# TIERS/multi-modal-loam

Hardware: AMD Instinct MI355X
Metric: scans/s (feature-extract+kNN+10 GN iters) on 16-ring x1800 + Livox 24k fused cloud (higher is better)
Workload: dtype f32/f64; 1 GPU; BASELINE configs[1]: fused VLP-16 16x1800 + Livox Horizon 24000 scan (52800 pts), local map 200000 pts, 1 association pass (thres_dist 25), 10 GN iterations, W=1; resident_slots=8192, stream_lanes=2, distinct_scans=64, map_tiles_touched=43, map_tiles_complete=43, parallelism=scan-sharded x1, device=AMD Radeon Graphics, cus=256

## Files before the change

### multi-modal-loam_amd/csrc/capi.hip

```cpp
#include <math.h>
#include <stdarg.h>
#include <stdio.h>
#include <stdlib.h>
#include <string.h>

#include <algorithm>

#include "mml_internal.h"

int mml_launch_detect_line(mml_ctx* ctx, int n, uint16_t* d_final);

namespace {

constexpr int kPackMaxSlots = 16;
constexpr size_t kStageDoubles = 1u << 22;

double* stage_alloc(mml_ctx* ctx, size_t doubles) {
    if (ctx->stage_cursor + doubles > ctx->h_stage_doubles) {
        mml_sync_all(ctx);
        ctx->stage_cursor = 0;
    }
    double* p = ctx->h_stage + ctx->stage_cursor;
    ctx->stage_cursor += (doubles + 7) & ~size_t(7);
    return p;
// ... 5 lines not shown
    if (e != hipSuccess) return e;
    ctx->cus = prop.multiProcessorCount;
    ctx->n_lanes = 2;
    if (const char* v = getenv("MML_LANES")) {
        const int n = atoi(v);
        if (n >= 1 && n <= mml_ctx::MAX_LANES) ctx->n_lanes = n;
    }
    const auto off = [](const char* name) {
        const char* v = getenv(name);
        return v && atoi(v) == 0;
    };
    ctx->onepass_wanted = !off("MML_ASSIGN_ONEPASS");
    ctx->solve_wide = !off("MML_SOLVE_WIDE");
    ctx->use_graph = getenv("MML_NO_GRAPH") == nullptr;
    ctx->lazy_undistort = !off("MML_LAZY_UNDISTORT");
    return hipSuccess;
}

}

double* mml_stage_alloc(mml_ctx* ctx, size_t doubles) { return stage_alloc(ctx, doubles); }

int mml_refuse(mml_ctx* ctx, int code, const char* fmt, ...) {
    if (ctx) {
        char m[192];
        va_list ap;
        va_start(ap, fmt);
        vsnprintf(m, sizeof(m), fmt, ap);
        va_end(ap);
        ctx->err = m;
// ... 79 lines not shown
    if (ctx->cfg.cell_surf <= 0) ctx->cfg.cell_surf = 5.0f * ctx->cfg.leaf_surf;
    if (ctx->cfg.max_features <= 0) ctx->cfg.max_features = 8192;
    if (ctx->cfg.max_map_points <= 0) ctx->cfg.max_map_points = 1 << 21;
    ctx->B = cfg->max_scans;
    ctx->NV = (cfg->max_velo_points + 63) & ~63;
    ctx->NL = (cfg->max_livox_points + 63) & ~63;
    ctx->NT = ctx->NV + ctx->NL;
    ctx->L = cfg->n_rings + cfg->n_livox_lines;
    ctx->MF = ctx->cfg.max_features;
    ctx->MM = ctx->cfg.max_map_points;
    ctx->VX_CAP = (int)ctx->NT;
    ctx->h_n_in.assign((size_t)ctx->B * 2, 0);
    ctx->raw_extracted.assign((size_t)ctx->B, 0);
    ctx->stats_stale.assign((size_t)ctx->B, 1);
    ctx->und_pending.assign((size_t)ctx->B, 0);
    auto fail = [&](hipError_t e, const char* what) {
        ctx->err = std::string(what) + ": " + hipGetErrorString(e);
        mml_destroy(ctx);
        return MML_ERR_HIP;
    };
    hipError_t e;
    if ((e = hipSetDevice(device)) != hipSuccess) return fail(e, "hipSetDevice");
    if ((e = read_settings(ctx)) != hipSuccess) return fail(e, "hipGetDeviceProperties");
    for (int l = 0; l < mml_ctx::MAX_LANES; ++l) {
        if ((e = hipStreamCreateWithFlags(&ctx->streams[l], hipStreamNonBlocking)) != hipSuccess)
            return fail(e, "hipStreamCreate");
        if ((e = hipEventCreateWithFlags(&ctx->lane_mark[l], hipEventDisableTiming)) != hipSuccess)
            return fail(e, "hipEventCreate");
    }
    if ((e = hipStreamCreateWithFlags(&ctx->copy_stream, hipStreamNonBlocking)) != hipSuccess) return fail(e, "hipStreamCreate");
// ... 650 lines not shown
int mml_cloud_download_registered(mml_ctx* ctx, int slot, const double* T_wl, uint8_t* out, int capacity_points, int* n_points) {
    return mml_cloud_download_registered_batch(ctx, slot, 1, T_wl, out, capacity_points, n_points);
}

int mml_cloud_upload(mml_ctx* ctx, int slot, const uint8_t* pointxyzinormal, int n_points, int n_velo) {
    CHECK_SLOTS(slot, 1);
    MML_REQUIRE(n_points >= 0 && n_velo >= 0 && n_velo <= n_points, MML_ERR_INVALID, "bad point counts");
    MML_REQUIRE(n_points == 0 || pointxyzinormal, MML_ERR_INVALID, "null point buffer");
    MML_REQUIRE(n_velo <= ctx->NV && n_points - n_velo <= ctx->NL, MML_ERR_CAPACITY,
                "cloud exceeds max_velo_points / max_livox_points (the Velodyne and Livox parts have their own regions)");
    const size_t bytes = (size_t)n_points * 48;
    int rc = ensure_wire_stage(ctx, bytes ? bytes : 48);
    if (rc != MML_OK) return rc;
    if (bytes) MML_HIP(hipMemcpyAsync(ctx->wire_stage.d, pointxyzinormal, bytes, hipMemcpyHostToDevice, MML_STREAM(ctx)));
    ctx->und_pending[slot] = 0;
    rc = mml_launch_cloud_decode(ctx, slot, reinterpret_cast<const float*>(ctx->wire_stage.d), n_points, n_velo);
    if (rc != MML_OK) return rc;
    MML_HIP(hipStreamSynchronize(MML_STREAM(ctx)));
    return MML_OK;
}

int mml_extract(mml_ctx* ctx, int first_slot, int count, const float* livox_extrinsic) {
    CHECK_SLOTS(first_slot, count);
    bool have = false;
    if (livox_extrinsic) {
        static const float I[16] = {1, 0, 0, 0, 0, 1, 0, 0, 0, 0, 1, 0, 0, 0, 0, 1};
        have = memcmp(I, livox_extrinsic, sizeof(I)) != 0;
        if (have) {
            double* st = stage_alloc(ctx, 8);
            memcpy(st, livox_extrinsic, sizeof(float) * 16);
// ... 1177 lines not shown
```

### multi-modal-loam_amd/csrc/feature.hip

```cpp
#include <math.h>

#include <algorithm>
#include <stdlib.h>

#include "libm_f32.h"
#include "mml_internal.h"

namespace {

enum : unsigned {
    A_W2 = 1u << 0,
    A_ANGLE = 1u << 1,
    A_CAND3 = 1u << 2,
    A_FAR = 1u << 3,
    A_REFL = 1u << 4,
    A_A3_SHIFT = 5,
    A_B3_SHIFT = 7,
    A_LFLAT = 1u << 9,
    A_RFLAT = 1u << 10,
    A_C150 = 1u << 11,
    A_F5_SHIFT = 12,
    A_NEAR = 1u << 14,
    A_VIS = 1u << 15
};
// ... 131 lines not shown
    }
    return ((unsigned long long)mhi << 32) | mlo;
}

typedef float v4f_nt __attribute__((ext_vector_type(4)));
__device__ __forceinline__ float4 nt_load4(const float4* p) {
    const v4f_nt v = __builtin_nontemporal_load(reinterpret_cast<const v4f_nt*>(p));
    return make_float4(v.x, v.y, v.z, v.w);
}

struct AssignAux {
    int first_finite, last_finite, trig, kept_velo;
    float startOri, endOri;
    int kept_livox, pad;
};
__device__ __forceinline__ void crop_test(const FeatParams& P, float x, float y, float z, bool& keep, bool& near_ok) {
    const float near2 = P.near_th * P.near_th, far2 = P.far_th * P.far_th;
    const float dis = x * x + y * y + z * z;
    keep = !(dis < near2 || dis > far2);
    near_ok = !(dis < near2);
}

__global__ void k_assign_init(FeatParams P, int count) {
    const int t = blockIdx.x * blockDim.x + threadIdx.x;
    if (t == 0) {
        P.sel_list_cnt[2 * P.first] = 0;
        P.sel_list_cnt[2 * P.first + 1] = 0;
    }
    if (t < count) {
        AssignAux* a = reinterpret_cast<AssignAux*>(P.assign_aux) + (P.first + t);
// ... 31 lines not shown
    const float guard = __builtin_fmaf(1.2e-4f, fabsf(inv_step), 2e-4f);
    const float rr = __builtin_fmaf(p.x, p.x, p.y * p.y);
    const float est = atan_est(p.z * __builtin_amdgcn_rsqf(rr)) * 57.29577951308232f;
    const float t = __builtin_fmaf(est - pitch0, inv_step, 0.5f);
    int scanID;
    if (fabsf(t - rintf(t)) > guard && fabsf(t) < 1e6f) {
        scanID = (int)t;
    } else {
        const float angle = (float)((double)(mml_libm::atanf_fd(p.z / sqrtf(p.x * p.x + p.y * p.y)) * 180.0f) / M_PI);
        const double v = (angle - pitch0) / pitch_step + 0.5;
        scanID = (v != v || v >= 2147483648.0 || v <= -2147483649.0) ? (-2147483647 - 1) : int(v);
    }
    return (scanID > (R - 1) || scanID < 0) ? 255 : scanID;
}

__device__ __forceinline__ float neg_atan2f(float y, float x) { return -mml_libm::atan2f_fd(y, x); }
__device__ __forceinline__ void sweep_azimuths(const float4 p0, const float4 p1, float& startOri, float& endOri) {
    startOri = neg_atan2f(p0.y, p0.x);
    endOri = (float)((double)neg_atan2f(p1.y, p1.x) + 2 * M_PI);
}

__global__ void k_libm_f32(const float* y, const float* x, long n, float* o2, float* o1) {
    const long i = (long)blockIdx.x * blockDim.x + threadIdx.x;
    if (i >= n) return;
    if (o2) o2[i] = mml_libm::atan2f_fd(y[i], x[i]);
    if (o1) o1[i] = mml_libm::atanf_fd(y[i]);
}

template <int PPT>
__global__ __launch_bounds__(AB_THREADS) void k_assign_a(FeatParams P) {
    __shared__ int s_bcnt[MAX_LINES];
// ... 285 lines not shown
    if (lane == 0) s_wvalid[wave] = __popcll(km);
    __syncthreads();
    if (!valid) return;
    const AssignAux* a = &aux;
    int pos = s_cnt[key] + __popcll(eq & lt);
    int fdst = (sensor == 0 ? 0 : a->kept_velo) + s_cnt[MAX_LINES + 1] + __popcll(km & lt);
    for (int w = 0; w < wave; ++w) {
        pos += s_wcnt[w][key];
        fdst += s_wvalid[w];
    }
    const int dst = s_ls[key] + pos;
    const size_t g = (size_t)b * P.NT + dst;
    P.ln_pts[g] = praw;
    float rel;
    if (sensor == 0) {
        const float startOri = a->startOri, endOri = a->endOri;
        float ori = P.raw_ori[(size_t)b * P.NV + i];
        if (i <= a->trig) {
            if (ori < startOri - M_PI / 2)
                ori += 2 * M_PI;
            else if (ori > startOri + M_PI * 3 / 2)
                ori -= 2 * M_PI;
        } else {
            ori += 2 * M_PI;
            if (ori < endOri - M_PI * 3 / 2)
                ori += 2 * M_PI;
            else if (ori > endOri + M_PI / 2)
                ori -= 2 * M_PI;
        }
        rel = (ori - startOri) / (endOri - startOri);
    } else {
        const mml_livox_point* in = P.livox_in + (size_t)b * P.NL;
        const double timeSpan = livox_to_sec(in[n - 1].offset_time);
        rel = livox_to_sec(off_time) / timeSpan;
    }
    P.ln_gidx[g] = keep ? fdst : ((sensor == 1 && near_ok) ? -2 : -1);
    P.ln_rel[g] = __float_as_int(rel);
}

#ifndef MML_CB_TP
#define MML_CB_TP 2
#endif
constexpr int CB_TP = MML_CB_TP;
constexpr int CB_THREADS = 1024;
constexpr int CB_TILE = CB_THREADS * CB_TP;
// ... 114 lines not shown
#pragma unroll
    for (int r = 0; r < CB_TP; ++r) {
        if (!valid[r]) continue;
        const int i = bx * CB_TILE + r * CB_THREADS + tid;
        const AssignAux* a = &aux;
        const int g = r * CB_WAVES + wave;
        const int sub = g / gpb;
        int pos = s_cnt[sub][key[r]] + rank[r];
        int fdst = (sensor == 0 ? 0 : a->kept_velo) + s_cnt[sub][MAX_LINES + 1] + krank[r];
        for (int w = sub * gpb; w < g; ++w) {
            pos += s_wcnt[w][key[r]];
            fdst += s_wvalid[w];
        }
        float rel;
        if (sensor == 0) {
            const float startOri = a->startOri, endOri = a->endOri;
            float o = ori[r];
            if (i <= a->trig) {
                if (o < startOri - M_PI / 2)
                    o += 2 * M_PI;
                else if (o > startOri + M_PI * 3 / 2)
                    o -= 2 * M_PI;
            } else {
                o += 2 * M_PI;
                if (o < endOri - M_PI * 3 / 2)
                    o += 2 * M_PI;
                else if (o > endOri + M_PI / 2)
                    o -= 2 * M_PI;
            }
            rel = (o - startOri) / (endOri - startOri);
        } else {
            rel = livox_to_sec(off_time[r]) / timeSpan;
        }
        const int e = s_kstart[key[r]] + (pos - s_cnt[0][key[r]]);
        s_pt[e] = praw[r];
        s_meta[e] = make_int2(keep[r] ? fdst : ((sensor == 1 && near_ok[r]) ? -2 : -1), __float_as_int(rel));
        s_dst[e] = s_ls[key[r]] + pos;
    }
    __syncthreads();
    const int nstaged = s_kstart[nkeys];
    for (int e = tid; e < nstaged; e += CB_THREADS) {
        const size_t g = (size_t)b * P.NT + s_dst[e];
        P.ln_pts[g] = s_pt[e];
        P.ln_gidx[g] = s_meta[e].x;
        P.ln_rel[g] = s_meta[e].y;
// ... 88 lines not shown
    return hipMemcpyFromSymbol(out, HIP_SYMBOL(g_op_dbg), sizeof(unsigned long long) * 16) == hipSuccess ? 0 : -1;
}
#else
#define OP_MARK(id)
#define OP_MARK0(id)
#endif
struct OnepassLds {
    int cnt[OP_GROUPS][OP_CSTRIDE];
    int gv[OP_GROUPS], gk[OP_GROUPS];
    int hist[OP_MAXKEYS + 2], koff[OP_MAXKEYS];
    int cond[OP_WAVES];
    int base[3];
    float ori[2];
    int out[2][MML_OP_BLK];
};
template <int SENSOR>
__device__ __forceinline__ void assign_onepass_body(const FeatParams& P, OnepassLds& S) {
    auto& s_cnt = S.cnt;
    auto& s_gv = S.gv;
    auto& s_gk = S.gk;
    auto& s_hist = S.hist;
    auto& s_koff = S.koff;
    auto& s_cond = S.cond;
    auto& s_base = S.base;
    auto& s_out = S.out;
    const int b = blockIdx.y + P.first, blk = blockIdx.x;
    const int tid = threadIdx.x, lane = tid & 63, wave = tid >> 6;
    const int i0 = blk * MML_OP_BLK;
#ifdef MML_OP_TIMING
    const bool op_dbg = SENSOR == 0 && tid == 64 && blk == MML_OP_TIMING && b == P.first + 517;
    const bool op_dbg0 = SENSOR == 0 && tid == 0 && blk == MML_OP_TIMING && b == P.first + 517;
    unsigned long long op_prev = clock64(), op_prev0 = op_prev;
// ... 10 lines not shown
        const mml_livox_point* in = P.livox_in + (size_t)b * P.NL;
#pragma unroll
        for (int r = 0; r < OP_PPT; ++r) {
            typedef unsigned lv_u4 __attribute__((ext_vector_type(4), aligned(4)));
            const unsigned* w = reinterpret_cast<const unsigned*>(in + min(i0 + r * OP_THREADS + tid, P.NL - 1));
            const lv_u4 head = *reinterpret_cast<const lv_u4*>(w);
            const unsigned tail = w[4];
            pt[r] = make_float4(__uint_as_float(head.y), __uint_as_float(head.z), __uint_as_float(head.w),
                                (float)(tail & 255u));
            xw[r] = head.x;
            info[r] = (tail >> 16) & 255u;
        }
    }
    const int n = P.n_in[2 * b + SENSOR];
    if (blk == 0 && tid == 0 && (SENSOR == 0 || P.n_in[2 * b] <= 0)) {
        P.slot_flags[2 * b] = 0;
        P.brk_cnt[b] = 0;
        P.redo_cnt[b] = 0;
    }
    if (i0 >= n) return;
    const int nkeys = SENSOR == 0 ? P.n_rings : P.n_lines;
    const int nbits = SENSOR == 0 ? P.ring_bits : P.line_bits;
    const int region = SENSOR == 0 ? 0 : P.NV;
    for (int k = tid; k < OP_GROUPS * OP_CSTRIDE; k += OP_THREADS) (&s_cnt[0][0])[k] = 0;
    if (SENSOR == 0 && wave == 0) {
        float so, eo;
        if (P.ends_inline) {
            sweep_ends(P, b, so, eo);
        } else {
            const AssignAux* a = reinterpret_cast<const AssignAux*>(P.assign_aux) + b;
            so = a->startOri;
            eo = a->endOri;
        }
        if (lane == 0) {
            S.ori[0] = so;
            S.ori[1] = eo;
        }
    }
    struct {
        float startOri, endOri;
    } aux;
    OP_MARK(0);
    __syncthreads();
    OP_MARK(1);
    aux.startOri = S.ori[0];
    aux.endOri = S.ori[1];
    const unsigned long long lt = (lane == 0) ? 0ull : (~0ull >> (64 - lane));
    int cond_min = 0x7fffffff;
#pragma unroll
    for (int r = 0; r < OP_PPT; ++r) {
        const int i = i0 + r * OP_THREADS + tid;
        bool valid = false, keep = false, near_ok = false, cond = false;
        int key = 0;
        if (i < n) {
            if constexpr (SENSOR == 0) {
                const float4 p = pt[r];
                float ori = 0.f;
                if (isfinite(p.x) && isfinite(p.y) && isfinite(p.z)) {
                    const int ring = velo_ring(p, P.pitch0, P.pitch_step, P.n_rings);
                    valid = ring != 255;
                    key = valid ? ring : 0;
                    ori = neg_atan2f(p.y, p.x);
                }
                xw[r] = __float_as_uint(ori);
                if (valid) {
                    float o = ori;
                    if (o < aux.startOri - M_PI / 2)
                        o += 2 * M_PI;
                    else if (o > aux.startOri + M_PI * 3 / 2)
                        o -= 2 * M_PI;
                    cond = o - aux.startOri > M_PI;
                }
            } else {
                const int line_num = (int)(info[r] & 255u);
                valid = !(line_num > nkeys - 1) && !(pt[r].x < 0.01);
                key = valid ? line_num : 0;
            }
            if (valid) crop_test(P, pt[r].x, pt[r].y, pt[r].z, keep, near_ok);
        }
        const unsigned long long eq = match_key(valid, key, nbits);
        const unsigned long long km = __ballot(keep), vm = __ballot(valid);
        const int g = r * OP_WAVES + wave;
        if (valid && (eq & lt) == 0) s_cnt[g][key] = __popcll(eq);
        if (lane == 0) {
            s_gv[g] = __popcll(vm);
            s_gk[g] = __popcll(km);
        }
// ... 104 lines not shown
    __syncthreads();
    OP_MARK(6);
    const int base_valid = region + s_base[0], base_keep = s_base[1], trig = s_base[2];
    double timeSpan = 1.0;
    if constexpr (SENSOR == 1) timeSpan = livox_to_sec(P.livox_in[(size_t)b * P.NL + n - 1].offset_time);
#pragma unroll
    for (int r = 0; r < OP_PPT; ++r) {
        const unsigned f = info[r];
        if (!(f & OPI_VALID)) continue;
        const int i = i0 + r * OP_THREADS + tid;
        const int key = (int)(f & 255u), g = r * OP_WAVES + wave;
        const int dst = base_valid + s_koff[key] + s_cnt[g][key] + (int)((f >> OPI_RANK_SHIFT) & 63u);
        const int fdst = base_keep + s_gk[g] + (int)((f >> OPI_KRANK_SHIFT) & 63u);
        float rel;
        if constexpr (SENSOR == 0) {
            const float startOri = aux.startOri, endOri = aux.endOri;
            float ori = __uint_as_float(xw[r]);
            if (i <= trig) {
                if (ori < startOri - M_PI / 2)
                    ori += 2 * M_PI;
                else if (ori > startOri + M_PI * 3 / 2)
                    ori -= 2 * M_PI;
            } else {
                ori += 2 * M_PI;
                if (ori < endOri - M_PI * 3 / 2)
                    ori += 2 * M_PI;
                else if (ori > endOri + M_PI / 2)
                    ori -= 2 * M_PI;
            }
            rel = (ori - startOri) / (endOri - startOri);
        } else {
            rel = livox_to_sec(xw[r]) / timeSpan;
        }
        const size_t gpos = (size_t)b * P.NT + dst;
        P.ln_pts[gpos] = pt[r];
        const bool keep = (f & OPI_KEEP) != 0;
        const int q = dst - base_valid;
        s_out[0][q] = keep ? fdst : ((SENSOR == 1 && (f & OPI_NEAR)) ? -2 : -1);
        s_out[1][q] = __float_as_int(rel);
        __builtin_amdgcn_sched_barrier(0);
    }
    OP_MARK(7);
    __syncthreads();
    OP_MARK(8);
    {
        const int tv = s_hist[nkeys];
        int* og = P.ln_gidx + (size_t)b * P.NT + base_valid;
        int* orl = P.ln_rel + (size_t)b * P.NT + base_valid;
        for (int k = tid; k < tv; k += OP_THREADS) {
            og[k] = s_out[0][k];
            orl[k] = s_out[1][k];
        }
    }
#ifdef MML_OP_TIMING
    asm volatile("s_waitcnt vmcnt(0)" ::: "memory");
    OP_MARK(9);
#endif
}

__global__ __launch_bounds__(OP_THREADS) void k_assign_onepass(FeatParams P) {
    __shared__ OnepassLds S;
    if (blockIdx.z == 0)
        assign_onepass_body<0>(P, S);
    else
        assign_onepass_body<1>(P, S);
}
template <int SENSOR>
__global__ __launch_bounds__(OP_THREADS) void k_assign_onepass_s(FeatParams P) {
    __shared__ OnepassLds S;
    assign_onepass_body<SENSOR>(P, S);
}

constexpr int TB_THREADS = 256;
__global__ __launch_bounds__(TB_THREADS) void k_assign_tables(FeatParams P, int count) {
    __shared__ int s_cum[64][MML_SEG_MAX + 1], s_pos[64][MML_SEG_MAX];
    __shared__ int s_nseg[64], s_len[64], s_rb[64];
    const int t = blockIdx.x;
    if (t >= count) return;
    const int b = P.first + t, tid = threadIdx.x;
    if (t == 0 && tid == 64) {
        P.sel_list_cnt[2 * P.first] = 0;
        P.sel_list_cnt[2 * P.first + 1] = 0;
    }
    if (tid < 64) {
        const int lane = tid;
// ... 2329 lines not shown
        return MML_ERR_HIP;
    float *dy = ty.d, *dx = tx.d, *d2 = t2.d, *d1 = t1.d;
    bool ok = hipMemcpy(dy, y, bytes, hipMemcpyHostToDevice) == hipSuccess && hipMemcpy(dx, x, bytes, hipMemcpyHostToDevice) == hipSuccess;
    if (ok) {
        hipLaunchKernelGGL(k_libm_f32, dim3((unsigned)((n + 255) / 256)), dim3(256), 0, MML_STREAM(ctx), dy, dx, n, d2, d1);
        ok = hipStreamSynchronize(MML_STREAM(ctx)) == hipSuccess;
    }
    if (ok && out_atan2) ok = hipMemcpy(out_atan2, d2, bytes, hipMemcpyDeviceToHost) == hipSuccess;
    if (ok && out_atan) ok = hipMemcpy(out_atan, d1, bytes, hipMemcpyDeviceToHost) == hipSuccess;
    return ok ? MML_OK : MML_ERR_HIP;
}

int mml_launch_extract(mml_ctx* ctx, int first, int count, bool have_extrinsic) {
    for (int i = 0; i < count; ++i) ctx->raw_extracted[first + i] = 1;
    for (int i = 0; i < count; ++i) ctx->und_pending[first + i] = 0;
    FeatParams P = make_params(ctx, first);
    P.extr = have_extrinsic ? ctx->d_extr : nullptr;
    hipStream_t s = MML_STREAM(ctx);
    if (ctx->onepass) {
        ctx->op_epoch = (ctx->op_epoch + 1) & 0x1ffffffu;
        if (ctx->op_epoch == 0) ctx->op_epoch = 1;
        P.op_epoch = ctx->op_epoch;
        const int nbv = (ctx->NV + MML_OP_BLK - 1) / MML_OP_BLK, nbl = (ctx->NL + MML_OP_BLK - 1) / MML_OP_BLK;
        P.ends_inline = count <= ST_SEGMENT_MAX_SLOTS ? 1 : 0;
        if (!P.ends_inline) {
            MmlStageScope t(ctx, "assign_ends");
            hipLaunchKernelGGL(k_assign_ends, dim3(count), dim3(64), 0, s, P, count);
        }
        {
            MmlStageScope t(ctx, "assign_onepass");
            const int nb = nbv > nbl ? nbv : nbl;
            if (P.ends_inline) {
                if (nb > 0) hipLaunchKernelGGL(k_assign_onepass, dim3(nb, count, nbl > 0 ? 2 : 1), dim3(OP_THREADS), 0, s, P);
            } else {
                if (nbv > 0) hipLaunchKernelGGL(k_assign_onepass_s<0>, dim3(nbv, count), dim3(OP_THREADS), 0, s, P);
                if (nbl > 0) hipLaunchKernelGGL(k_assign_onepass_s<1>, dim3(nbl, count), dim3(OP_THREADS), 0, s, P);
            }
        }
        {
            MmlStageScope t(ctx, "assign_tables");
            hipLaunchKernelGGL(k_assign_tables, dim3(count), dim3(TB_THREADS), 0, s, P, count);
        }
    } else {
    {
        MmlStageScope t(ctx, "assign_count");
        hipLaunchKernelGGL(k_assign_init, dim3((count + 255) / 256), dim3(256), 0, s, P, count);
        if (P.ab_ppt == 4)
            hipLaunchKernelGGL((k_assign_a<4>), dim3(P.nblk_max, count, 2), dim3(AB_THREADS), 0, s, P);
        else
            hipLaunchKernelGGL((k_assign_a<1>), dim3(P.nblk_max, count, 2), dim3(AB_THREADS), 0, s, P);
    }
    {
// ... 178 lines not shown
```

### multi-modal-loam_amd/csrc/mml_internal.h

```cpp
#ifndef MML_INTERNAL_H
#define MML_INTERNAL_H

#include <hip/hip_runtime.h>
#include <stdint.h>

#include <string>
#include <vector>

#include "mml_mem.h"
#include "mmloam_hip.h"

#define MML_WAVE 64

namespace mml_und {
__device__ __forceinline__ double sconst(double v) {
    asm("" : "+s"(v));
    return v;
}
}
#define MML_SEG_MAX 16
#define MML_OP_BLK 4096
#define MML_SEG_FLAT 512
#define MML_VOXEL_LDS_CAP 8192

// ... 57 lines not shown
    struct WinGraph {
        int first, count, W, max_iters, fixed;
        double huber, w_tan;
        hipStream_t stream;
        const double* Tbl;
        bool second;
        hipGraphExec_t exec;
    };
    std::vector<WinGraph> win_graphs;
    int device = 0;
    int cus = 0;
    bool onepass_wanted = true;
    bool solve_wide = true;
    bool use_graph = true;
    bool lazy_undistort = true;
    static constexpr int MAX_LANES = 8;
    hipStream_t streams[MAX_LANES] = {};
    hipStream_t copy_stream = nullptr;
    hipEvent_t lane_mark[MAX_LANES] = {};
    struct Upload {
        int first, count;
        hipEvent_t done;
    };
    std::vector<Upload> uploads;
    std::vector<hipEvent_t> upload_event_pool;
    int n_lanes = 1;
    int cur = 0;
    std::string err;
    MmlFixed fixed;

// ... 37 lines not shown
    unsigned* brk_queue = nullptr;
    int* brk_cnt = nullptr;
    int* queue_off = nullptr;
    unsigned* redo_queue = nullptr;
    uint8_t* sel_done = nullptr;
    int* sel_list = nullptr;
    int* sel_list_cnt = nullptr;
    unsigned char* st_exit = nullptr;
    int* vx_big = nullptr;

    int* cb_n = nullptr;

    uint8_t* ln_line = nullptr;
    int* slot_flags = nullptr;
    std::vector<char> und_pending;
    uint8_t* ln_label = nullptr;
    int* fu_info = nullptr;

    float4* ft_xyz[2] = {nullptr, nullptr};
    int* ft_n = nullptr;
    unsigned long long* vx_keys = nullptr;
    int* vx_gidx = nullptr;
    unsigned long long* seg_keys = nullptr;
    unsigned* seg_vals = nullptr;
    float4* seg_cat = nullptr;
    int* seg_flag = nullptr;
    int* seg_meta = nullptr;
    MmlGroup seg_scratch;
    MmlStaging<char, false> seg_tmp[8];
    int VX_CAP = 0;
// ... 116 lines not shown
int mml_stage_begin(mml_ctx* ctx, const char* name);
void mml_stage_end(mml_ctx* ctx, int token);
struct MmlStageScope {
    mml_ctx* c;
    int t;
    MmlStageScope(mml_ctx* ctx, const char* name) : c(ctx), t(mml_stage_begin(ctx, name)) {}
    ~MmlStageScope() { mml_stage_end(c, t); }
};

int mml_launch_extract(mml_ctx* ctx, int first, int count, bool have_extrinsic);
int mml_launch_cloud_decode(mml_ctx* ctx, int slot, const float* d_raw, int n, int n_velo);
int mml_launch_undistort(mml_ctx* ctx, int first, int count, const double* d_params);
int mml_launch_undistort_listed(mml_ctx* ctx, int first, int count, const double* d_params);
int mml_cloud_settle(mml_ctx* ctx, int first, int count);
#define MML_LABEL_SETTLED 0x40
int mml_launch_downsample(mml_ctx* ctx, int first, int count);
inline int mml_voxel_cap_corner(const mml_ctx* ctx) { return (ctx->NT > 65536 || MML_VOXEL_LDS_CAP < 2048) ? MML_VOXEL_LDS_CAP : 2048; }
int mml_build_grid(mml_ctx* ctx, int kind, const float* h_xyz, int m);
int mml_build_grid_device(mml_ctx* ctx, int kind, int m);
int mml_downsample_big(mml_ctx* ctx, int first, int count);
int mml_downsample_redo_overflow(mml_ctx* ctx, int first, int count, std::vector<int>* redone);
int mml_map_upkeep_increment(mml_ctx* ctx, int slot, const double* T_wl, int* n_out);
int mml_build_global_grid(mml_ctx* ctx, int kind, const float* h_xyz, const int* h_cube, int m, const int* cen);
int mml_build_global_grid_device(mml_ctx* ctx, int kind, const float4* d_pts, const uint16_t* d_tags, const int* d_cnt, int m,
                                 const int* cen);
int mml_cube_store_append(mml_ctx* ctx, int slot, const double* T_wl);
int mml_cube_store_increment(mml_ctx* ctx, const double* T_wl, int* n_out);
int mml_cube_store_download(mml_ctx* ctx, int kind, float* xyz, int* cube, int capacity, int* n, int* cen);
int mml_cube_store_reset(mml_ctx* ctx);
int mml_launch_knn5(mml_ctx* ctx, int kind, const float* d_q, int nq, float max_d2, int* d_idx, float* d_d2);
// ... 25 lines not shown
```

### multi-modal-loam_amd/csrc/undistort_dev.h

```cpp
#ifndef MML_UNDISTORT_DEV_H
#define MML_UNDISTORT_DEV_H
#include <hip/hip_runtime.h>
#include <math.h>

#include "mml_internal.h"

namespace mml_und {

struct Q4 {
    double x, y, z, w;
};
struct V3 {
    double x, y, z;
};
__device__ __forceinline__ V3 v3(double x, double y, double z) { return V3{x, y, z}; }
__device__ __forceinline__ V3 vcross(const V3& a, const V3& b) {
    return v3(a.y * b.z - a.z * b.y, a.z * b.x - a.x * b.z, a.x * b.y - a.y * b.x);
}
__device__ __forceinline__ double qdot(const Q4& a, const Q4& b) {
    return (a.x * b.x + a.z * b.z) + (a.y * b.y + a.w * b.w);
}
__device__ __forceinline__ Q4 qnormalized(const Q4& q) {
    double n = sqrt(qdot(q, q));
    return Q4{q.x / n, q.y / n, q.z / n, q.w / n};
// ... 149 lines not shown
```

### multi-modal-loam_amd/csrc/undistort_voxel.hip

```cpp
#include <math.h>

#include "mml_internal.h"
#include "undistort_dev.h"

namespace {
using namespace mml_und;

__global__ void k_undistort_prep(int count, const double* params, double* derived, double* par_keep, int* flags ) {
    const int s = blockIdx.x * blockDim.x + threadIdx.x;
    if (s >= count) return;
    for (int k = 0; k < 12; ++k) par_keep[12 * s + k] = params[12 * s + k];
    flags[2 * s + 1] = flags[2 * s];
    flags[2 * s] |= 2;
    const double* dR = params + 12 * s;
    const Q4 qlc = qnormalized(quat_from_matrix(dR));
    const double dd = (0.0 * qlc.x + 0.0 * qlc.z) + (0.0 * qlc.y + 1.0 * qlc.w);
    const double absD = fabs(dd);
    const double one = 1.0 - 2.220446049250313e-16;
    double theta = 0, sinTheta = 1;
    const bool linear = absD >= one;
    if (!linear) {
        theta = acos(absD);
        sinTheta = sin(theta);
    }
// ... 35 lines not shown
    __builtin_nontemporal_store(outv, pp);
}

constexpr int UND_LISTED_G = 8;
__device__ __forceinline__ int listed_position(const int* fu_info, const unsigned* lists, int list_stride, int NT, int b, int e) {
    const int nc = min(max(fu_info[8 * b + 6], 0), list_stride), ns = min(max(fu_info[8 * b + 7], 0), list_stride);
    if (e >= nc + ns) return -1;
    const int kind = e >= nc ? 1 : 0;
    const unsigned pos = lists[((size_t)b * 2 + kind) * list_stride + (e - (kind ? nc : 0))];
    return pos < (unsigned)NT ? (int)pos : -1;
}
__device__ __forceinline__ int listed_total(const int* fu_info, int list_stride, int b) {
    return min(max(fu_info[8 * b + 6], 0), list_stride) + min(max(fu_info[8 * b + 7], 0), list_stride);
}

__global__ __launch_bounds__(256) void k_undistort_listed(int first, int NT, int list_stride, const int* fu_info, const unsigned* lists,
                                                         float4* ln_pts, const int* ln_rel, const int* slot_flags, const double* params,
                                                         const double* derived) {
    const int b = blockIdx.y + first;
    const int n = listed_total(fu_info, list_stride, b);
    const bool time_is_one = (slot_flags[2 * b + 1] & 2) != 0;
    const double* dR = params + 12 * blockIdx.y;
    for (int e = blockIdx.x * 256 + threadIdx.x; e < n; e += UND_LISTED_G * 256) {
        const int pos = listed_position(fu_info, lists, list_stride, NT, b, e);
        if (pos < 0) continue;
        float4 p = ln_pts[(size_t)b * NT + pos];
        const float s = time_is_one ? 1.0f : __int_as_float(ln_rel[(size_t)b * NT + pos]);
        mml_und::undistort_point(dR, dR + 9, derived + 8 * blockIdx.y, s, p);
        ln_pts[(size_t)b * NT + pos] = p;
    }
}

__global__ __launch_bounds__(256) void k_settle_mark(int first, int NT, int list_stride, const int* fu_info, const unsigned* lists,
                                                    uint8_t* ln_label) {
    const int b = blockIdx.y + first;
    const int n = listed_total(fu_info, list_stride, b);
    for (int e = blockIdx.x * 256 + threadIdx.x; e < n; e += UND_LISTED_G * 256) {
        const int pos = listed_position(fu_info, lists, list_stride, NT, b, e);
        if (pos < 0) continue;
        uint8_t* lab = ln_label + (size_t)b * NT + pos;
        *lab = (uint8_t)(*lab | MML_LABEL_SETTLED);
    }
}

#ifdef MML_VX_TIMING
__device__ unsigned long long g_vx_dbg[16];
#define VX_MARK(id)                                    \
    do {                                               \
        if (vx_dbg) {                                  \
            const unsigned long long now_ = clock64(); \
            g_vx_dbg[id] += now_ - vx_prev;            \
            vx_prev = now_;                            \
        }                                              \
    } while (0)
extern "C" int mml_debug_vx_timing(unsigned long long* out, int reset) {
    if (reset) {
        unsigned long long z[16] = {};
// ... 370 lines not shown
    const int cap = blockIdx.y == 0 ? A.cap_y0 : A.cap_y1;
    if constexpr (LIST) {
        const int nbig = A.big[A.first];
        for (int e = blockIdx.x; e < nbig; e += gridDim.x) {
            voxel_slot<VX_THREADS>(A, S, keys, __builtin_amdgcn_readfirstlane(A.big[A.B + A.first + e]), kind, cap);
            __syncthreads();
        }
    } else {
        if (A.zero_big && blockIdx.x == 0 && blockIdx.y == 0 && threadIdx.x == 0) A.big[A.first] = 0;
        voxel_slot<VX_THREADS>(A, S, keys, (int)blockIdx.x + A.first, kind, cap);
    }
}

}

int mml_launch_undistort(mml_ctx* ctx, int first, int count, const double* d_params) {
    MmlStageScope t(ctx, "undistort");
    dim3 grid((ctx->NT + 255) / 256, count);
    hipLaunchKernelGGL(k_undistort_prep, dim3((count + 63) / 64), dim3(64), 0, MML_STREAM(ctx), count, d_params, ctx->d_und + 8 * (size_t)first,
                       ctx->d_und_par + 12 * (size_t)first, ctx->slot_flags + 2 * (size_t)first);
    hipLaunchKernelGGL(k_undistort<false>, grid, dim3(256), 0, MML_STREAM(ctx), first, ctx->NT, ctx->NV, ctx->cb_n, ctx->ln_pts,
                       ctx->ln_rel, ctx->slot_flags, d_params, ctx->d_und + 8 * (size_t)first, (uint8_t*)nullptr);
    MML_HIP(hipGetLastError());
    return MML_OK;
}

int mml_launch_undistort_listed(mml_ctx* ctx, int first, int count, const double* d_params) {
    MmlStageScope t(ctx, "undistort");
    for (int i = 0; i < count; ++i) ctx->und_pending[first + i] = 1;
    hipLaunchKernelGGL(k_undistort_prep, dim3((count + 63) / 64), dim3(64), 0, MML_STREAM(ctx), count, d_params, ctx->d_und + 8 * (size_t)first,
                       ctx->d_und_par + 12 * (size_t)first, ctx->slot_flags + 2 * (size_t)first);
    hipLaunchKernelGGL(k_undistort_listed, dim3(UND_LISTED_G, count), dim3(256), 0, MML_STREAM(ctx), first, ctx->NT, ctx->VX_CAP, ctx->fu_info,
                       reinterpret_cast<const unsigned*>(ctx->vx_keys), ctx->ln_pts, ctx->ln_rel, ctx->slot_flags, d_params,
                       ctx->d_und + 8 * (size_t)first);
    MML_HIP(hipGetLastError());
    return MML_OK;
}

int mml_cloud_settle(mml_ctx* ctx, int first, int count) {
    for (int i = 0; i < count;) {
        if (!ctx->und_pending[first + i]) {
            ++i;
            continue;
        }
        int n = 1;
        while (i + n < count && ctx->und_pending[first + i + n] && n < 32768) ++n;
        const int f = first + i;
        MmlStageScope t(ctx, "undistort_settle");
        hipLaunchKernelGGL(k_settle_mark, dim3(UND_LISTED_G, n), dim3(256), 0, MML_STREAM(ctx), f, ctx->NT, ctx->VX_CAP, ctx->fu_info,
                           reinterpret_cast<const unsigned*>(ctx->vx_keys), ctx->ln_label);
        hipLaunchKernelGGL(k_undistort<true>, dim3((ctx->NT + 255) / 256, n), dim3(256), 0, MML_STREAM(ctx), f, ctx->NT, ctx->NV, ctx->cb_n,
                           ctx->ln_pts, ctx->ln_rel, ctx->slot_flags, ctx->d_und_par + 12 * (size_t)f, ctx->d_und + 8 * (size_t)f, ctx->ln_label);
        MML_HIP(hipGetLastError());
        for (int k = 0; k < n; ++k) ctx->und_pending[f + k] = 0;
        i += n;
    }
    return MML_OK;
}

int mml_launch_downsample(mml_ctx* ctx, int first, int count) {
    MmlStageScope t(ctx, "voxel_downsample");
    for (int i = 0; i < count; ++i) ctx->stats_stale[first + i] = 1;
    if (ctx->NT > (1 << 20)) return mml_downsample_big(ctx, first, count);
    const int cap_surf = MML_VOXEL_LDS_CAP, cap_corner = mml_voxel_cap_corner(ctx);
    auto lds = [](int cap) { return (size_t)cap * sizeof(unsigned long long); };
    VoxelArgs A;
    A.first = first;
    A.NT = ctx->NT;
    A.MF = ctx->MF;
    A.B = ctx->B;
    A.list_stride = ctx->VX_CAP;
    A.fu_info = ctx->fu_info;
// ... 39 lines not shown
```

Before: 437,900 scans/s.

## Defer exact Velodyne azimuth and relative-time computation to undistortion points

In the one-pass ring assignment, a cheap polynomial atan2 estimate with reciprocal approximation decides the half-sweep flag. The exact atan2 is computed only when the estimate is near a decision boundary. Per-point relative time is no longer computed there; only the half-turn bit is stored and the slot is flagged as pending. The exact time is then computed lazily, only for listed points during undistortion, or in a new materialise kernel before full or settle undistortion. This removes exact atan2 work for every raw point at the cost of extra state, a flag protocol, and an added kernel on the settle path.

Result: no change. 440,900 scans/s (median of 6 runs) (+0.7%).

```diff
diff --git a/multi-modal-loam_amd/csrc/azimuth_est.h b/multi-modal-loam_amd/csrc/azimuth_est.h
--- /dev/null
+++ b/multi-modal-loam_amd/csrc/azimuth_est.h
@@ -0,0 +1,46 @@
+#pragma once
+#if defined(__HIPCC__)
+#define MML_AZI_HD __host__ __device__ inline __attribute__((always_inline))
+#else
+#define MML_AZI_HD inline
+#endif
+
+namespace mml_azi {
+
+constexpr float AZI_EST_ERR = 7.2e-7f;
+constexpr float AZI_GUARD = 4e-6f;
+
+MML_AZI_HD bool azimuth_est_defined(float y, float x) {
+    const float m = __builtin_fmaxf(__builtin_fabsf(x), __builtin_fabsf(y));
+    return m > 1e-18f && m < 1e18f;
+}
+
+template <class RCP>
+MML_AZI_HD float atan2f_est(float y, float x, RCP rcp) {
+    const float ax = __builtin_fabsf(x), ay = __builtin_fabsf(y);
+    const bool swap = ay > ax;
+    const float t = (swap ? ax : ay) * rcp(swap ? ay : ax);
+    const float z = t * t;
+    float p = -0.004054564982652664f;
+    p = __builtin_fmaf(p, z, 0.021862952038645744f);
+    p = __builtin_fmaf(p, z, -0.0559123232960701f);
+    p = __builtin_fmaf(p, z, 0.0964219719171524f);
+    p = __builtin_fmaf(p, z, -0.1390862911939621f);
+    p = __builtin_fmaf(p, z, 0.19946566224098206f);
+    p = __builtin_fmaf(p, z, -0.33329859375953674f);
+    p = __builtin_fmaf(p, z, 0.9999993443489075f);
+    float r = p * t;
+    r = swap ? 1.57079637f - r : r;
+    r = x < 0.0f ? 3.14159274f - r : r;
+    return __builtin_copysignf(r, y);
+}
+
+MML_AZI_HD bool half_turn_from_estimate(float est, float startOri, float t1, float t2, bool& cond) {
+    const float d1 = est - t1, d2 = est - t2;
+    const float w = est + (d1 < 0.0f ? 6.28318548f : (d2 > 0.0f ? -6.28318548f : 0.0f));
+    const float d3 = (w - startOri) - 3.14159274f;
+    cond = d3 > 0.0f;
+    return __builtin_fabsf(d1) > AZI_GUARD && __builtin_fabsf(d2) > AZI_GUARD && __builtin_fabsf(d3) > AZI_GUARD;
+}
+
+}
diff --git a/multi-modal-loam_amd/csrc/capi.hip b/multi-modal-loam_amd/csrc/capi.hip
--- a/multi-modal-loam_amd/csrc/capi.hip
+++ b/multi-modal-loam_amd/csrc/capi.hip
@@ -43,6 +43,10 @@
     ctx->solve_wide = !off("MML_SOLVE_WIDE");
     ctx->use_graph = getenv("MML_NO_GRAPH") == nullptr;
     ctx->lazy_undistort = !off("MML_LAZY_UNDISTORT");
+    {
+        const char* v = getenv("MML_EXACT_AZIMUTH");
+        ctx->exact_azimuth = v && atoi(v) != 0;
+    }
     return hipSuccess;
 }
 
@@ -152,6 +156,7 @@
     ctx->raw_extracted.assign((size_t)ctx->B, 0);
     ctx->stats_stale.assign((size_t)ctx->B, 1);
     ctx->und_pending.assign((size_t)ctx->B, 0);
+    ctx->azi_pending.assign((size_t)ctx->B, 0);
     auto fail = [&](hipError_t e, const char* what) {
         ctx->err = std::string(what) + ": " + hipGetErrorString(e);
         mml_destroy(ctx);
@@ -832,6 +837,7 @@
     if (rc != MML_OK) return rc;
     if (bytes) MML_HIP(hipMemcpyAsync(ctx->wire_stage.d, pointxyzinormal, bytes, hipMemcpyHostToDevice, MML_STREAM(ctx)));
     ctx->und_pending[slot] = 0;
+    ctx->azi_pending[slot] = 0;
     rc = mml_launch_cloud_decode(ctx, slot, reinterpret_cast<const float*>(ctx->wire_stage.d), n_points, n_velo);
     if (rc != MML_OK) return rc;
     MML_HIP(hipStreamSynchronize(MML_STREAM(ctx)));
diff --git a/multi-modal-loam_amd/csrc/feature.hip b/multi-modal-loam_amd/csrc/feature.hip
--- a/multi-modal-loam_amd/csrc/feature.hip
+++ b/multi-modal-loam_amd/csrc/feature.hip
@@ -1,10 +1,13 @@
 #include <math.h>
+#include <stddef.h>
 
 #include <algorithm>
 #include <stdlib.h>
 
+#include "azimuth_est.h"
 #include "libm_f32.h"
 #include "mml_internal.h"
+#include "undistort_dev.h"
 
 namespace {
 
@@ -169,6 +172,9 @@
     float startOri, endOri;
     int kept_livox, pad;
 };
+static_assert(offsetof(AssignAux, startOri) == 4 * MML_AUX_START_ORI && offsetof(AssignAux, endOri) == 4 * (MML_AUX_START_ORI + 1) &&
+                  sizeof(AssignAux) == 4 * MML_AUX_INTS,
+              "undistort_voxel.hip reads the sweep's two azimuths from assign_aux by these offsets");
 __device__ __forceinline__ void crop_test(const FeatParams& P, float x, float y, float z, bool& keep, bool& near_ok) {
     const float near2 = P.near_th * P.near_th, far2 = P.far_th * P.far_th;
     const float dis = x * x + y * y + z * z;
@@ -230,7 +236,8 @@
     return (scanID > (R - 1) || scanID < 0) ? 255 : scanID;
 }
 
-__device__ __forceinline__ float neg_atan2f(float y, float x) { return -mml_libm::atan2f_fd(y, x); }
+using mml_und::neg_atan2f;
+using mml_und::velo_rel_time;
 __device__ __forceinline__ void sweep_azimuths(const float4 p0, const float4 p1, float& startOri, float& endOri) {
     startOri = neg_atan2f(p0.y, p0.x);
     endOri = (float)((double)neg_atan2f(p1.y, p1.x) + 2 * M_PI);
@@ -546,21 +553,7 @@
     P.ln_pts[g] = praw;
     float rel;
     if (sensor == 0) {
-        const float startOri = a->startOri, endOri = a->endOri;
-        float ori = P.raw_ori[(size_t)b * P.NV + i];
-        if (i <= a->trig) {
-            if (ori < startOri - M_PI / 2)
-                ori += 2 * M_PI;
-            else if (ori > startOri + M_PI * 3 / 2)
-                ori -= 2 * M_PI;
-        } else {
-            ori += 2 * M_PI;
-            if (ori < endOri - M_PI * 3 / 2)
-                ori += 2 * M_PI;
-            else if (ori > endOri + M_PI / 2)
-                ori -= 2 * M_PI;
-        }
-        rel = (ori - startOri) / (endOri - startOri);
+        rel = velo_rel_time(P.raw_ori[(size_t)b * P.NV + i], i > a->trig, a->startOri, a->endOri);
     } else {
         const mml_livox_point* in = P.livox_in + (size_t)b * P.NL;
         const double timeSpan = livox_to_sec(in[n - 1].offset_time);
@@ -705,21 +698,7 @@
         }
         float rel;
         if (sensor == 0) {
-            const float startOri = a->startOri, endOri = a->endOri;
-            float o = ori[r];
-            if (i <= a->trig) {
-                if (o < startOri - M_PI / 2)
-                    o += 2 * M_PI;
-                else if (o > startOri + M_PI * 3 / 2)
-                    o -= 2 * M_PI;
-            } else {
-                o += 2 * M_PI;
-                if (o < endOri - M_PI * 3 / 2)
-                    o += 2 * M_PI;
-                else if (o > endOri + M_PI / 2)
-                    o -= 2 * M_PI;
-            }
-            rel = (o - startOri) / (endOri - startOri);
+            rel = velo_rel_time(ori[r], i > a->trig, a->startOri, a->endOri);
         } else {
             rel = livox_to_sec(off_time[r]) / timeSpan;
         }
@@ -838,8 +817,9 @@
     float ori[2];
     int out[2][MML_OP_BLK];
 };
-template <int SENSOR>
+template <int SENSOR, bool LAZY>
 __device__ __forceinline__ void assign_onepass_body(const FeatParams& P, OnepassLds& S) {
+    static_assert(SENSOR == 0 || !LAZY, "Livox records are not touched by the lazy azimuth");
     auto& s_cnt = S.cnt;
     auto& s_gv = S.gv;
     auto& s_gk = S.gk;
@@ -880,7 +860,7 @@
     }
     const int n = P.n_in[2 * b + SENSOR];
     if (blk == 0 && tid == 0 && (SENSOR == 0 || P.n_in[2 * b] <= 0)) {
-        P.slot_flags[2 * b] = 0;
+        P.slot_flags[2 * b] = LAZY ? MML_SLOT_AZI_PENDING : 0;
         P.brk_cnt[b] = 0;
         P.redo_cnt[b] = 0;
     }
@@ -901,6 +881,11 @@
         if (lane == 0) {
             S.ori[0] = so;
             S.ori[1] = eo;
+            if (LAZY && P.ends_inline && blk == 0) {
+                AssignAux* a = reinterpret_cast<AssignAux*>(P.assign_aux) + b;
+                a->startOri = so;
+                a->endOri = eo;
+            }
         }
     }
     struct {
@@ -911,6 +896,7 @@
     OP_MARK(1);
     aux.startOri = S.ori[0];
     aux.endOri = S.ori[1];
+    const float thr1 = (float)((double)aux.startOri - M_PI / 2), thr2 = (float)((double)aux.startOri + M_PI * 3 / 2);
     const unsigned long long lt = (lane == 0) ? 0ull : (~0ull >> (64 - lane));
     int cond_min = 0x7fffffff;
 #pragma unroll
@@ -926,17 +912,23 @@
                     const int ring = velo_ring(p, P.pitch0, P.pitch_step, P.n_rings);
                     valid = ring != 255;
                     key = valid ? ring : 0;
-                    ori = neg_atan2f(p.y, p.x);
+                    bool decided = false;
+                    if constexpr (LAZY) {
+                        const float est = -mml_azi::atan2f_est(p.y, p.x, [](float v) { return __builtin_amdgcn_rcpf(v); });
+                        decided = mml_azi::half_turn_from_estimate(est, aux.startOri, thr1, thr2, cond) && mml_azi::azimuth_est_defined(p.y, p.x);
+                    }
+                    if (!decided && (valid || !LAZY)) {
+                        ori = neg_atan2f(p.y, p.x);
+                        float o = ori;
+                        if (o < aux.startOri - M_PI / 2)
+                            o += 2 * M_PI;
+                        else if (o > aux.startOri + M_PI * 3 / 2)
+                            o -= 2 * M_PI;
+                        cond = o - aux.startOri > M_PI;
+                    }
+                    cond = cond && valid;
                 }
-                xw[r] = __float_as_uint(ori);
-                if (valid) {
-                    float o = ori;
-                    if (o < aux.startOri - M_PI / 2)
-                        o += 2 * M_PI;
-                    else if (o > aux.startOri + M_PI * 3 / 2)
-                        o -= 2 * M_PI;
-                    cond = o - aux.startOri > M_PI;
-                }
+                if constexpr (!LAZY) xw[r] = __float_as_uint(ori);
             } else {
                 const int line_num = (int)(info[r] & 255u);
                 valid = !(line_num > nkeys - 1) && !(pt[r].x < 0.01);
@@ -1071,21 +1063,10 @@
         const int fdst = base_keep + s_gk[g] + (int)((f >> OPI_KRANK_SHIFT) & 63u);
         float rel;
         if constexpr (SENSOR == 0) {
-            const float startOri = aux.startOri, endOri = aux.endOri;
-            float ori = __uint_as_float(xw[r]);
-            if (i <= trig) {
-                if (ori < startOri - M_PI / 2)
-                    ori += 2 * M_PI;
-                else if (ori > startOri + M_PI * 3 / 2)
-                    ori -= 2 * M_PI;
-            } else {
-                ori += 2 * M_PI;
-                if (ori < endOri - M_PI * 3 / 2)
-                    ori += 2 * M_PI;
-                else if (ori > endOri + M_PI / 2)
-                    ori -= 2 * M_PI;
-            }
-            rel = (ori - startOri) / (endOri - startOri);
+            if constexpr (LAZY)
+                rel = __int_as_float(i > trig ? 1 : 0);
+            else
+                rel = velo_rel_time(__uint_as_float(xw[r]), i > trig, aux.startOri, aux.endOri);
         } else {
             rel = livox_to_sec(xw[r]) / timeSpan;
         }
@@ -1115,17 +1096,18 @@
 #endif
 }
 
+template <bool LAZY>
 __global__ __launch_bounds__(OP_THREADS) void k_assign_onepass(FeatParams P) {
     __shared__ OnepassLds S;
     if (blockIdx.z == 0)
-        assign_onepass_body<0>(P, S);
+        assign_onepass_body<0, LAZY>(P, S);
     else
-        assign_onepass_body<1>(P, S);
-}
-template <int SENSOR>
+        assign_onepass_body<1, false>(P, S);
+}
+template <int SENSOR, bool LAZY = false>
 __global__ __launch_bounds__(OP_THREADS) void k_assign_onepass_s(FeatParams P) {
     __shared__ OnepassLds S;
-    assign_onepass_body<SENSOR>(P, S);
+    assign_onepass_body<SENSOR, LAZY>(P, S);
 }
 
 constexpr int TB_THREADS = 256;
@@ -3485,6 +3467,7 @@
 int mml_launch_extract(mml_ctx* ctx, int first, int count, bool have_extrinsic) {
     for (int i = 0; i < count; ++i) ctx->raw_extracted[first + i] = 1;
     for (int i = 0; i < count; ++i) ctx->und_pending[first + i] = 0;
+    for (int i = 0; i < count; ++i) ctx->azi_pending[first + i] = 0;
     FeatParams P = make_params(ctx, first);
     P.extr = have_extrinsic ? ctx->d_extr : nullptr;
     hipStream_t s = MML_STREAM(ctx);
@@ -3501,12 +3484,15 @@
         {
             MmlStageScope t(ctx, "assign_onepass");
             const int nb = nbv > nbl ? nbv : nbl;
+            const bool lazy = !ctx->exact_azimuth;
             if (P.ends_inline) {
-                if (nb > 0) hipLaunchKernelGGL(k_assign_onepass, dim3(nb, count, nbl > 0 ? 2 : 1), dim3(OP_THREADS), 0, s, P);
+                if (nb > 0) hipLaunchKernelGGL((lazy ? k_assign_onepass<true> : k_assign_onepass<false>), dim3(nb, count, nbl > 0 ? 2 : 1), dim3(OP_THREADS), 0, s, P);
             } else {
-                if (nbv > 0) hipLaunchKernelGGL(k_assign_onepass_s<0>, dim3(nbv, count), dim3(OP_THREADS), 0, s, P);
-                if (nbl > 0) hipLaunchKernelGGL(k_assign_onepass_s<1>, dim3(nbl, count), dim3(OP_THREADS), 0, s, P);
-            }
+                if (nbv > 0) hipLaunchKernelGGL((lazy ? k_assign_onepass_s<0, true> : k_assign_onepass_s<0, false>), dim3(nbv, count), dim3(OP_THREADS), 0, s, P);
+                if (nbl > 0) hipLaunchKernelGGL((k_assign_onepass_s<1, false>), dim3(nbl, count), dim3(OP_THREADS), 0, s, P);
+            }
+            if (lazy && nbv > 0)
+                for (int i = 0; i < count; ++i) ctx->azi_pending[first + i] = 1;
         }
         {
             MmlStageScope t(ctx, "assign_tables");
diff --git a/multi-modal-loam_amd/csrc/mml_internal.h b/multi-modal-loam_amd/csrc/mml_internal.h
--- a/multi-modal-loam_amd/csrc/mml_internal.h
+++ b/multi-modal-loam_amd/csrc/mml_internal.h
@@ -95,6 +95,7 @@
     bool solve_wide = true;
     bool use_graph = true;
     bool lazy_undistort = true;
+    bool exact_azimuth = false;
     static constexpr int MAX_LANES = 8;
     hipStream_t streams[MAX_LANES] = {};
     hipStream_t copy_stream = nullptr;
@@ -162,6 +163,7 @@
     uint8_t* ln_line = nullptr;
     int* slot_flags = nullptr;
     std::vector<char> und_pending;
+    std::vector<char> azi_pending;
     uint8_t* ln_label = nullptr;
     int* fu_info = nullptr;
 
@@ -308,6 +310,9 @@
 int mml_launch_undistort_listed(mml_ctx* ctx, int first, int count, const double* d_params);
 int mml_cloud_settle(mml_ctx* ctx, int first, int count);
 #define MML_LABEL_SETTLED 0x40
+#define MML_SLOT_AZI_PENDING 4
+#define MML_AUX_INTS 8
+#define MML_AUX_START_ORI 4
 int mml_launch_downsample(mml_ctx* ctx, int first, int count);
 inline int mml_voxel_cap_corner(const mml_ctx* ctx) { return (ctx->NT > 65536 || MML_VOXEL_LDS_CAP < 2048) ? MML_VOXEL_LDS_CAP : 2048; }
 int mml_build_grid(mml_ctx* ctx, int kind, const float* h_xyz, int m);
diff --git a/multi-modal-loam_amd/csrc/undistort_dev.h b/multi-modal-loam_amd/csrc/undistort_dev.h
--- a/multi-modal-loam_amd/csrc/undistort_dev.h
+++ b/multi-modal-loam_amd/csrc/undistort_dev.h
@@ -3,9 +3,30 @@
 #include <hip/hip_runtime.h>
 #include <math.h>
 
+#include "libm_f32.h"
 #include "mml_internal.h"
 
 namespace mml_und {
+
+__device__ __forceinline__ float velo_rel_time(float ori, bool half_passed, float startOri, float endOri) {
+    if (!half_passed) {
+        if (ori < startOri - M_PI / 2)
+            ori += 2 * M_PI;
+        else if (ori > startOri + M_PI * 3 / 2)
+            ori -= 2 * M_PI;
+    } else {
+        ori += 2 * M_PI;
+        if (ori < endOri - M_PI * 3 / 2)
+            ori += 2 * M_PI;
+        else if (ori > endOri + M_PI / 2)
+            ori -= 2 * M_PI;
+    }
+    return (ori - startOri) / (endOri - startOri);
+}
+__device__ __forceinline__ float neg_atan2f(float y, float x) { return -mml_libm::atan2f_fd(y, x); }
+__device__ __forceinline__ float velo_time_from_point(const float4& p, int half_bit, float startOri, float endOri) {
+    return velo_rel_time(neg_atan2f(p.y, p.x), half_bit != 0, startOri, endOri);
+}
 
 struct Q4 {
     double x, y, z, w;
diff --git a/multi-modal-loam_amd/csrc/undistort_voxel.hip b/multi-modal-loam_amd/csrc/undistort_voxel.hip
--- a/multi-modal-loam_amd/csrc/undistort_voxel.hip
+++ b/multi-modal-loam_amd/csrc/undistort_voxel.hip
@@ -73,18 +73,26 @@
     return min(max(fu_info[8 * b + 6], 0), list_stride) + min(max(fu_info[8 * b + 7], 0), list_stride);
 }
 
-__global__ __launch_bounds__(256) void k_undistort_listed(int first, int NT, int list_stride, const int* fu_info, const unsigned* lists,
-                                                         float4* ln_pts, const int* ln_rel, const int* slot_flags, const double* params,
-                                                         const double* derived) {
+__global__ __launch_bounds__(256) void k_undistort_listed(int first, int NT, int NV, int list_stride, const int* fu_info, const unsigned* lists,
+                                                         float4* ln_pts, int* ln_rel, const int* slot_flags, const int* assign_aux,
+                                                         const double* params, const double* derived) {
     const int b = blockIdx.y + first;
     const int n = listed_total(fu_info, list_stride, b);
-    const bool time_is_one = (slot_flags[2 * b + 1] & 2) != 0;
+    const int fl = slot_flags[2 * b + 1];
+    const bool time_is_one = (fl & 2) != 0, azi_pending = (fl & MML_SLOT_AZI_PENDING) != 0;
+    const float startOri = __int_as_float(assign_aux[MML_AUX_INTS * b + MML_AUX_START_ORI]);
+    const float endOri = __int_as_float(assign_aux[MML_AUX_INTS * b + MML_AUX_START_ORI + 1]);
     const double* dR = params + 12 * blockIdx.y;
     for (int e = blockIdx.x * 256 + threadIdx.x; e < n; e += UND_LISTED_G * 256) {
         const int pos = listed_position(fu_info, lists, list_stride, NT, b, e);
         if (pos < 0) continue;
         float4 p = ln_pts[(size_t)b * NT + pos];
-        const float s = time_is_one ? 1.0f : __int_as_float(ln_rel[(size_t)b * NT + pos]);
+        float s = __int_as_float(ln_rel[(size_t)b * NT + pos]);
+        if (azi_pending && pos < NV) {
+            s = velo_time_from_point(p, __float_as_int(s), startOri, endOri);
+            ln_rel[(size_t)b * NT + pos] = __float_as_int(s);
+        }
+        if (time_is_one) s = 1.0f;
         mml_und::undistort_point(dR, dR + 9, derived + 8 * blockIdx.y, s, p);
         ln_pts[(size_t)b * NT + pos] = p;
     }
@@ -100,6 +108,22 @@
         uint8_t* lab = ln_label + (size_t)b * NT + pos;
         *lab = (uint8_t)(*lab | MML_LABEL_SETTLED);
     }
+}
+
+__global__ __launch_bounds__(256) void k_velo_times(int first, int NT, const int* cb_n, const float4* ln_pts, int* ln_rel, int* slot_flags,
+                                                   const int* assign_aux, const uint8_t* ln_label) {
+    const int b = blockIdx.y + first;
+    const int i = blockIdx.x * 256 + threadIdx.x;
+    if (i == 0) {
+        slot_flags[2 * b] &= ~MML_SLOT_AZI_PENDING;
+        slot_flags[2 * b + 1] &= ~MML_SLOT_AZI_PENDING;
+    }
+    if (i >= cb_n[2 * b]) return;
+    const size_t g = (size_t)b * NT + i;
+    if (ln_label[g] & MML_LABEL_SETTLED) return;
+    const float startOri = __int_as_float(assign_aux[MML_AUX_INTS * b + MML_AUX_START_ORI]);
+    const float endOri = __int_as_float(assign_aux[MML_AUX_INTS * b + MML_AUX_START_ORI + 1]);
+    ln_rel[g] = __float_as_int(velo_time_from_point(ln_pts[g], ln_rel[g], startOri, endOri));
 }
 
 #ifdef MML_VX_TIMING
@@ -500,7 +524,30 @@
 
 }
 
+static int velo_times_materialise(mml_ctx* ctx, int first, int count) {
+    if (ctx->NV <= 0) return MML_OK;
+    for (int i = 0; i < count;) {
+        if (!ctx->azi_pending[first + i]) {
+            ++i;
+            continue;
+        }
+        int n = 1;
+        while (i + n < count && ctx->azi_pending[first + i + n] && n < 32768) ++n;
+        const int f = first + i;
+        hipLaunchKernelGGL(k_velo_times, dim3((ctx->NV + 255) / 256, n), dim3(256), 0, MML_STREAM(ctx), f, ctx->NT, ctx->cb_n, ctx->ln_pts,
+                           ctx->ln_rel, ctx->slot_flags, ctx->assign_aux, ctx->ln_label);
+        MML_HIP(hipGetLastError());
+        for (int k = 0; k < n; ++k) ctx->azi_pending[f + k] = 0;
+        i += n;
+    }
+    return MML_OK;
+}
+
 int mml_launch_undistort(mml_ctx* ctx, int first, int count, const double* d_params) {
+    {
+        const int rc = velo_times_materialise(ctx, first, count);
+        if (rc != MML_OK) return rc;
+    }
     MmlStageScope t(ctx, "undistort");
     dim3 grid((ctx->NT + 255) / 256, count);
     hipLaunchKernelGGL(k_undistort_prep, dim3((count + 63) / 64), dim3(64), 0, MML_STREAM(ctx), count, d_params, ctx->d_und + 8 * (size_t)first,
@@ -516,9 +563,9 @@
     for (int i = 0; i < count; ++i) ctx->und_pending[first + i] = 1;
     hipLaunchKernelGGL(k_undistort_prep, dim3((count + 63) / 64), dim3(64), 0, MML_STREAM(ctx), count, d_params, ctx->d_und + 8 * (size_t)first,
                        ctx->d_und_par + 12 * (size_t)first, ctx->slot_flags + 2 * (size_t)first);
-    hipLaunchKernelGGL(k_undistort_listed, dim3(UND_LISTED_G, count), dim3(256), 0, MML_STREAM(ctx), first, ctx->NT, ctx->VX_CAP, ctx->fu_info,
-                       reinterpret_cast<const unsigned*>(ctx->vx_keys), ctx->ln_pts, ctx->ln_rel, ctx->slot_flags, d_params,
-                       ctx->d_und + 8 * (size_t)first);
+    hipLaunchKernelGGL(k_undistort_listed, dim3(UND_LISTED_G, count), dim3(256), 0, MML_STREAM(ctx), first, ctx->NT, ctx->NV, ctx->VX_CAP,
+                       ctx->fu_info, reinterpret_cast<const unsigned*>(ctx->vx_keys), ctx->ln_pts, ctx->ln_rel, ctx->slot_flags, ctx->assign_aux,
+                       d_params, ctx->d_und + 8 * (size_t)first);
     MML_HIP(hipGetLastError());
     return MML_OK;
 }
@@ -535,13 +582,17 @@
         MmlStageScope t(ctx, "undistort_settle");
         hipLaunchKernelGGL(k_settle_mark, dim3(UND_LISTED_G, n), dim3(256), 0, MML_STREAM(ctx), f, ctx->NT, ctx->VX_CAP, ctx->fu_info,
                            reinterpret_cast<const unsigned*>(ctx->vx_keys), ctx->ln_label);
+        {
+            const int rc = velo_times_materialise(ctx, f, n);
+            if (rc != MML_OK) return rc;
+        }
         hipLaunchKernelGGL(k_undistort<true>, dim3((ctx->NT + 255) / 256, n), dim3(256), 0, MML_STREAM(ctx), f, ctx->NT, ctx->NV, ctx->cb_n,
                            ctx->ln_pts, ctx->ln_rel, ctx->slot_flags, ctx->d_und_par + 12 * (size_t)f, ctx->d_und + 8 * (size_t)f, ctx->ln_label);
         MML_HIP(hipGetLastError());
         for (int k = 0; k < n; ++k) ctx->und_pending[f + k] = 0;
         i += n;
     }
-    return MML_OK;
+    return velo_times_materialise(ctx, first, count);
 }
 
 int mml_launch_downsample(mml_ctx* ctx, int first, int count) {
```
